# szlhl1040/Vehicles-Dispatch-Simulator

Measured on AMD Instinct MI355X. Metric: env-steps x replicas / sec (192-cluster, 10k vehicles), higher is better.
Workload: dtype int32

## Files before the change

### vehicles_dispatch_simulator_amd/csrc/vds_api.hip

```cpp
#include "../../include/vds.h"
#include "../../include/vds_debug.h"
#include "vds_device.h"
#include "vds_launch.h"

#include <algorithm>
#include <unordered_map>
#include <atomic>
#include <chrono>
#include <thread>
#include <cstdarg>
#include <cstdio>
#include <cstdlib>
#include <cstring>
#include <exception>
#include <map>
#include <mutex>
#include <new>
#include <numeric>
#include <string>
#include <vector>
#include <execinfo.h>
#include <signal.h>
#include <unistd.h>

// ... 1338 lines not shown
            for (int dd = 0; dd < n_days; ++dd) ok = ok && PD[dd].npull == ddesc[dd].Oq;
        if (!ok && S.dense_st) { S.dense = 0; S.dense_st = 0; }
        if (!ok) S.pull = 0;
        else {
            struct Sink2 { vds_handle *h; ~Sink2() { h->alloc_sink = nullptr; } } sink2{h};
            h->alloc_sink = &h->order_allocs;
            S.pull_W = W; S.pull_hmax = hmax;
            if ((rc = upload(h, &d, so_slot))) return rc; S.so_slot = d;
            int2 *d2; if ((rc = upload(h, &d2, d_rec))) return rc; S.d_rec = d2;
            if ((rc = upload(h, &d, d_first))) return rc; S.d_first = d;
            h->pull_desc = ddesc2;
            d_first_keep = d_first;
            h->pull_drec = std::move(d_rec);
            h->pull_slot_q.assign(h->pull_drec.size(), 0);
            for_each_day(n_days, [&](int dd) {
                const int qb = ddesc[dd].q_base;
                for (int q = qb; q < qb + ddesc[dd].Oq; ++q)
                    if (so_slot[q] >= 0) h->pull_slot_q[(size_t)ddesc2[dd].y + so_slot[q]] = q - qb;
            });
        }
    }
    h->pull_Od_max = Od_max;
    lt.lap("static arrival slots");
    S.tdesc = nullptr;
    if (S.dense && n_days == 1 && (int)h->corder_host.size() == C) {
        const DayDesc &de = ddesc[0];
        std::vector<int4> td((size_t)std::max(de.T, 1) * C * 2, make_int4(0, 0, 0, 0));
        std::vector<int4> cdd((size_t)C);
        HIPCHK(h, hipMemcpy(cdd.data(), S.cdesc_dense, (size_t)C * sizeof(int4), hipMemcpyDeviceToHost));
        for (int t = 0; t < de.T; ++t)
            for (int ci = 0; ci < C; ++ci) {
                const int c = h->corder_host[ci];
                const int q0 = bkt_off[de.bkt_base + (size_t)t * C + c], k = bkt_off[de.bkt_base + (size_t)t * C + c + 1] - q0;
                int clo = 0, n = 0;
                if (S.pull) {
                    clo = d_first_keep[(size_t)std::max(t - S.pull_W, 0) * C + c];
                    n = d_first_keep[(size_t)(t + 1) * C + c] - clo;
                }
                td[2 * ((size_t)t * C + ci)] = make_int4(q0, k, clo, n);
                td[2 * ((size_t)t * C + ci) + 1] = cdd[ci];
            }
        struct Sink3 { vds_handle *h; ~Sink3() { h->alloc_sink = nullptr; } } sink3{h};
        h->alloc_sink = &h->order_allocs;
        int4 *dtd; if ((rc = upload(h, &dtd, td))) return rc; S.tdesc = dtd;
    }
    h->alloc_sink = nullptr;
    lt.lap("bucket descriptors");
    if ((rc = apply_replica_map(h))) return rc;
    h->alloc_sink = nullptr;
    h->alloc_O = (int)std::min<long long>(Ototal / n_days, 0x7fffffff);
    if ((rc = alloc_state(h, h->alloc_O))) return rc;
    lt.lap("state tables");
    {
        const Static &Z = h->S;
        const int ids2 = std::max(Z.max_tick_orders, 4 * Z.C);
        const size_t lds2 = ((size_t)9 * Z.C + 1 + ids2 + ((size_t)Z.V + 2) / 2) * sizeof(int) + 2048;
        h->dfs2_ok = h->dfs_mode && Omax <= (1 << 20) && Z.max_nc <= 2047 && h->cost_min >= 0 && h->cost_max < (1 << 15) &&
                     Z.V <= 20480 && Z.N <= 65534 && Z.C <= 3072 && h->blk_ints < (1ll << 29) && Z.idle_cap <= 32767 && Z.max_tick_orders < 32768 &&
                     lds2 <= 64 * 1024;
        h->S.walk_pool = 0; h->S.walk_pool = dfs_walk_pool(h->S);
        h->hybrid_ok = h->dfs_mode && h->cfg.force_generic == 0 && Z.fast_ok && Z.max_nc * Z.max_nc <= h->lds_ints &&
                       Z.max_tick_orders < 65535 && Z.V < 65536 && Z.max_nc <= 2047 &&
                       Z.N <= 65534 && Z.C <= 65535 && Z.idle_cap <= 16384 && h->cost_max < (1 << 15) && h->max_seq <= 256 &&
                       dfs_walk_lds(Z) + 1024 <= 64 * 1024 && Z.so_vis != nullptr;
        if (Z.dense_st && !h->hybrid_ok)
            return fail(h, VDS_ECAPACITY, "vds_load_orders: neighbour search on the dense layout needs the walk's tables (idle_cap %d <= 16384, %zu bytes of LDS <= 64 KB); VDS_DENSE_DFS=0 keeps the wide layout",
                        Z.idle_cap, dfs_walk_lds(Z) + 1024);
// ... 1442 lines not shown
```

### vehicles_dispatch_simulator_amd/csrc/vds_device.h

```cpp
#pragma once
#include <hip/hip_runtime.h>
#include <stdint.h>

namespace vds {

enum {
    HDR_IDLE = 0,
    HDR_IDLE_PRE = 1,
    HDR_ORDERS = 2,
    HDR_FL = 3,
    HDR_INBOX0 = 4,
    HDR_INBOX1 = 5,
    HDR_RAW = 6,
    HDR_CNT32 = 8,
    HDR_WORDS = 16
};

enum {
    CNT_ORDERS = 0, CNT_REJECTS = 1, CNT_WAIT = 2, CNT_VALUE = 3,
    CNT_EVALS = 4, CNT_ARRIVALS = 5, CNT_DISPATCH = 6, CNT_DISPATCH_COST = 7, CNT_WORDS = 8
};

enum { ERR_IDLE_CAP = 1, ERR_FL_CAP = 2, ERR_INBOX_CAP = 4, ERR_DISPATCH = 8, ERR_RING_CAP = 16 };

// ... 67 lines not shown
    const unsigned char *so_lb;
    int seq_pad;
    const int *so_rank;
    int max_tick_orders;
    int r_lo;
    int dense;
    int dense_lpr;
    int dense_tab, dense_keys;
    int dense_force_slow;
    const Static *self_dev;
    const struct State *state_dev;
    int pull, pull_W, pull_hmax;
    int arr_slots;
    const int *so_slot;
    const int2 *d_rec;
    const int *d_first;
    const int4 *replica_desc2;
    int ring_min_on;
    const int *blk32s;
    const unsigned char *blk8s;
    const int4 *cdesc_dense;
    int dense_st;
    const int4 *tdesc;
};

struct Emit {
    hipStream_t st = nullptr;
    hipGraph_t graph = nullptr;
    const hipGraphNode_t *deps = nullptr;
    size_t ndeps = 0;
    hipGraphNode_t *node = nullptr;
    hipError_t *err = nullptr;
};
template <typename T> struct emit_arg { using type = T; };
template <typename... P>
static inline void emit_kernel(const Emit &e, void (*k)(P...), dim3 grid, dim3 block, size_t lds, typename emit_arg<P>::type... a) {
    if (!e.graph) { hipLaunchKernelGGL(k, grid, block, lds, e.st, a...); return; }
    void *args[] = {(void *)&a...};
    hipKernelNodeParams p{};
    p.func = reinterpret_cast<void *>(k); p.gridDim = grid; p.blockDim = block; p.sharedMemBytes = (unsigned)lds; p.kernelParams = args; p.extra = nullptr;
    *e.err = hipGraphAddKernelNode(e.node, e.graph, e.deps, e.ndeps, &p);
}

struct State {
    int *hdr;
    long long *cnt;
    uint2 *idle;
    int4 *ring;
    int *ring_cnt;
    int4 *fl;
    int4 *inbox;
    int4 *slog;
    int2 *out;
    int *err;
    int *work;
    unsigned *arr;
    unsigned short *stamp;
    int *slow_tick;
    int slow_T;
    int *dry;
    int *sup;
    int *sup_slot;
    int *ring_min;
};

#define DENSE_PULL_WMAX 3
#define VDS_SUP_PLANES 32
__host__ __device__ inline size_t sup_index(int C, int R, int slot, int c, int r) { return ((size_t)(slot & (VDS_SUP_PLANES - 1)) * C + c) * R + r; }
__host__ __device__ inline size_t arr_index(int R, int slot, int r) { return (size_t)slot * (size_t)R + (size_t)r; }
__host__ __device__ inline unsigned pull_entry(int veh, int arrival_slot) { return ((unsigned)veh << 8) | ((unsigned)arrival_slot & 0xFFu); }
__host__ __device__ inline unsigned pull_reject(int t) { return 0xFFFFFF00u | ((unsigned)(t + 128) & 0xFFu); }
__host__ __device__ inline bool pull_is_reject(unsigned e) { return (e >> 8) == 0xFFFFFFu; }
__host__ __device__ inline int pull_slots_ahead(unsigned e, int now_slot) { return (int)(signed char)((e & 0xFFu) - ((unsigned)now_slot & 0xFFu)); }
#define DENSE_DEAD_COST 0x00FFFFFF
#define DENSE_ID_BITS 25
__host__ __device__ inline unsigned dense_pack(unsigned veh, unsigned loc) { return (veh << 8) | (loc & 0xFFu); }
__host__ __device__ inline unsigned dense_key(int tick, int is_dispatch, int id) {
    return ((unsigned)(tick & 63) << 26) | ((unsigned)(is_dispatch & 1) << 25) | ((unsigned)id & ((1u << DENSE_ID_BITS) - 1));
}
__host__ __device__ inline unsigned dense_key_rel(unsigned key, int t) { return key - ((unsigned)((t - 32) & 63) << 26); }
__host__ __device__ inline int dense_key_is_dispatch(unsigned key) { return (int)((key >> 25) & 1u); }
__host__ __device__ inline int dense_key_id(unsigned key) { return (int)(key & ((1u << DENSE_ID_BITS) - 1)); }
__host__ __device__ inline int dense_key_tick(unsigned key, int t_now) { return t_now - (int)(((unsigned)t_now - (key >> 26)) & 63u); }

struct IdleRef {
    uint2 *p;
    unsigned *q;
    __device__ __forceinline__ uint2 get(int e) const {
        if (!q) return p[e];
// ... 29 lines not shown
```

### vehicles_dispatch_simulator_amd/csrc/vds_tick_dense.hip

```cpp
#include "vds_kernels_common.h"
#include "vds_launch.h"
#include <algorithm>

namespace vds {

VDS_PROF_ACCESSORS(dense)

#define SPAN_TICKS 256
#ifdef VDS_PROF
#define SPAN_WAYS 64
static __device__ unsigned long long g_span[2 * SPAN_TICKS * SPAN_WAYS * 2];
void read_span_dense(unsigned long long *out, int reset, hipStream_t st) {
    (void)hipStreamSynchronize(st);
    static unsigned long long host[2 * SPAN_TICKS * SPAN_WAYS * 2];
    if (out) {
        (void)hipMemcpyFromSymbol(host, HIP_SYMBOL(g_span), sizeof(host));
        for (int i = 0; i < 2 * SPAN_TICKS; ++i) {
            unsigned long long lo = ~0ull, hi = 0ull;
            for (int w = 0; w < SPAN_WAYS; ++w) { lo = std::min(lo, host[(i * SPAN_WAYS + w) * 2]); hi = std::max(hi, host[(i * SPAN_WAYS + w) * 2 + 1]); }
            out[2 * i] = lo; out[2 * i + 1] = hi;
        }
    }
    if (reset) {
        for (int i = 0; i < 2 * SPAN_TICKS * SPAN_WAYS; ++i) { host[2 * i] = ~0ull; host[2 * i + 1] = 0ull; }
// ... 2 lines not shown
}
#else
void read_span_dense(unsigned long long *, int, hipStream_t) { }
#endif

#define DN_ROWS 16
#define DN_TAB 128
#define DN_KEYS 64
#define DN_ORDERS 64
#ifndef DN_ROWS32
#define DN_ROWS32 1
#endif
#define DN_TPAD 4

struct DenseArgs {
    int *hdr; long long *cnt; unsigned *idle; uint2 *ring; int *ring_cnt; int4 *inbox; int2 *out; int *err;
    const int4 *cdesc_dense; const char *blk; const int4 *so_rec; const int *bkt_off; const int4 *replica_desc; const int *rperm;
    int R, C, H, idle_cap, ring_cap, in_cap, Oq, arr_slots;
    int tick_minutes, now0, tick_div_limit; unsigned tick_magic;
    int r_lo, r_hi, dense_tab, dense_keys, dense_force_slow;
    int *ring_min;
    unsigned *arr; const int *so_slot; const int2 *d_rec; const int *d_first; const int4 *replica_desc2; int pull_W;
    const int4 *tdesc;
    unsigned short *stamp; int *dry; int *slow_tick; const int *so_rank;
    int slow_T;
    const int2 *bmap;
    int *sup, *sup_slot;
    const Static *Sdev; const State *Ddev;
};
__device__ __forceinline__ uint2 *ring2(const DenseArgs &D) { return D.ring; }
__device__ __forceinline__ int ticks_until_fast(const DenseArgs &S, int rel) {
    const int n = rel + S.tick_minutes - 1;
    if (S.tick_div_limit > (1 << 26)) return (int)__umulhi((unsigned)n, S.tick_magic);
    return n / S.tick_minutes;
}

template <int LPR>
__device__ __forceinline__ int grp_min(int v) {
    v = min(v, dpp_mov<0xB1, 0xF>(v, v));
    v = min(v, dpp_mov<0x4E, 0xF>(v, v));
    if (LPR >= 8) v = min(v, dpp_mov<0x141, 0xF>(v, v));
    if (LPR >= 16) v = min(v, dpp_mov<0x140, 0xF>(v, v));
    return v;
}
template <int LPR>
__device__ __forceinline__ int grp_max(int v) {
// ... 482 lines not shown
            if (J >= 4) {
#pragma unroll
                for (int s = 0; s < J; s += 4) *reinterpret_cast<uint4 *>(tab + lbase + s) = make_uint4(e[s], e[s + 1], e[s + 2], e[s + 3]);
            } else {
                *reinterpret_cast<uint2 *>(tab + lbase) = make_uint2(e[0], e[1]);
            }
        }
        wave_order();
    }
#pragma unroll
    for (int a = 0; a < NAP; ++a)
        if (a * LPR + lg < A) tab[m + rank[a]] = ent[a];
    wave_order();
}
template <int LPR, int J>
__device__ __forceinline__ void pull_rank_place_any(const uint2 *ring, unsigned *tab, const int2 *drec, int lg, int m, int Ac, int A, int Amax, unsigned tbase, const unsigned *e,
                                                    bool cmp = false, unsigned am = 0u, int wp0 = 0) {
    if (Amax <= LPR) pull_rank_place<LPR, 1, J>(ring, tab, drec, lg, m, Ac, A, Amax, tbase, e, cmp, am, wp0);
    else if (Amax <= 2 * LPR) pull_rank_place<LPR, 2, J>(ring, tab, drec, lg, m, Ac, A, Amax, tbase, e, cmp, am, wp0);
    else if (Amax <= 4 * LPR || LPR == 16) pull_rank_place<LPR, 4, J>(ring, tab, drec, lg, m, Ac, A, Amax, tbase, e, cmp, am, wp0);
    else pull_rank_place<LPR, 8, J>(ring, tab, drec, lg, m, Ac, A, Amax, tbase, e, cmp, am, wp0);
}

template <int LPR>
__device__ __forceinline__ void store_counters(long long *cnt, int lg, long long cntv, int k, int rej, int wsum, int vsum, int evals, int A) {
#pragma unroll
    for (int w0 = 0; w0 < CNT_WORDS; w0 += LPR) {
        const int w = w0 + lg;
        long long d = 0;
        if (w == CNT_ORDERS) d = k;
        if (w == CNT_REJECTS) d = rej;
        if (w == CNT_WAIT) d = wsum;
        if (w == CNT_VALUE) d = vsum;
        if (w == CNT_EVALS) d = evals;
        if (w == CNT_ARRIVALS) d = A;
        if (LPR >= CNT_WORDS) { if (w < CNT_WORDS && d != 0) cnt[w] = cntv + d; }
        else if (d != 0) cnt[w] += d;
    }
}

template <bool RAW = false>
__device__ __forceinline__ void store_record(int *hdr, int lg, int2 hw, int idle, int pre, int orders, int rej, int wsum, int vsum, int evals, int A, int raw = 0) {
    if (lg == 0) hw = make_int2(idle, pre);
    if (lg == 1) hw.x = orders;
    if (RAW && lg == 3) hw.x = raw;
    if (lg == 4) { hw.x += orders; hw.y += rej; }
// ... 34 lines not shown
    for (int s = 0; s < J; ++s) e[s] = 0u;
    const bool dl = ST && m_raw != m;
    const bool anydl = ST && ballot(dl) != 0ull;
    if ((kmax > 0 || anydl) && lbase < (ST ? m_raw : m) && !(abl & 2048)) {
        if (J >= 4) {
#pragma unroll
            for (int s = 0; s < J; s += 4) {
                const uint4 v = *reinterpret_cast<const uint4 *>(idle + lbase + s);
                e[s] = v.x; e[s + 1] = v.y; e[s + 2] = v.z; e[s + 3] = v.w;
            }
        } else {
            const uint2 v = *reinterpret_cast<const uint2 *>(idle + lbase);
            e[0] = v.x; e[1] = v.y;
        }
    }
    PROF_STAMP(3);
    const int Amax = (abl & 2048) ? 0 : wave_max_of_groups<LPR>(PULL ? Aring : A);
    const int Ntot = PULL ? ((abl & 2048) ? 0 : wave_max_of_groups<LPR>(A)) : Amax;
#ifdef VDS_PROF
    if ((g_ablate & 2097152) && lane == 0) { atomicAdd(&D.err[12], 1); if (Ntot > 4 * LPR) atomicAdd(&D.err[13], 1); if (Ntot > 8 * LPR) atomicAdd(&D.err[14], 1); if (TS == 128) atomicAdd(&D.err[15], 1); }
#endif
    const unsigned tbase = (unsigned)((t - 32) & 63) << 26;
    const uint2 *ring = ring2(D) + si * S.ring_cap;
    unsigned am = 0u;
    if (ST) {
        const int nv = min(max(m_raw - lbase, 0), J);
        am = nv >= 32 ? 0xFFFFFFFFu : ((1u << nv) - 1u);
        if (dl && lbase < m_raw) {
            const unsigned *sp = reinterpret_cast<const unsigned *>(D.stamp + b * S.idle_cap + lbase);
            unsigned sw[(J + 1) / 2];
            if (J >= 8) {
#pragma unroll
                for (int s = 0; s < J / 2; s += 4) { const uint4 v = *reinterpret_cast<const uint4 *>(sp + s); sw[s] = v.x; sw[s + 1] = v.y; sw[s + 2] = v.z; sw[s + 3] = v.w; }
            } else if (J == 4) { const uint2 v = *reinterpret_cast<const uint2 *>(sp); sw[0] = v.x; sw[1] = v.y; }
            else sw[0] = sp[0];
            unsigned fm = 0u;
#pragma unroll
            for (int s = 0; s < J; ++s) fm |= (((sw[s >> 1] >> ((s & 1) << 4)) & 0xFFFFu) == 0xFFFFu ? 1u : 0u) << s;
            am &= fm;
        }
    }
    if (kmax == 0 && !anydl) {
        if (Ntot > 0) {
            if (PULL) pull_rank_place_any<LPR, 0>(ring, tab, lds_drec, lg, 0, A - Aring, A, Ntot, tbase, nullptr);
            else merge_arrivals_any<LPR, 0>(ring, tab, lg, 0, A, Amax, tbase, nullptr);
            if (rowvalid) {
                for (int idx = lg; idx < A; idx += LPR) { idle[m + idx] = tab[idx]; if (ST) D.stamp[b * S.idle_cap + m + idx] = (unsigned short)0xFFFFu; }
                if (lg == 0 && (PULL ? Aring : A) > 0) D.ring_cnt[si] = 0;
            }
        }
        if (rowvalid && lg == 2 && D.sup != nullptr) D.sup[(size_t)(t & (VDS_SUP_PLANES - 1)) * S.C * S.R + b] = 0;
        if (rowvalid) {
            if (REC && ST) store_record<true>(D.hdr + b * HDR_WORDS, lg, hw, mnew, mnew, 0, 0, 0, 0, 0, A, 0);
            else if (REC) store_record(D.hdr + b * HDR_WORDS, lg, hw, mnew, mnew, 0, 0, 0, 0, 0, A);
            else {
                if (lg < 3) D.hdr[b * HDR_WORDS + lg] = lg == HDR_ORDERS ? 0 : mnew;
                if (A > 0) store_counters<LPR>(D.cnt + b * CNT_WORDS, lg, cntv, 0, 0, 0, 0, 0, A);
            }
        }
        return;
    }
    int fdl = IMAX;
    if (ST && anydl) {
        const int na = __popc(am);
        const int wp0 = grp_incl_scan<LPR>(na, lg) - na;
        const int nv = min(max(m_raw - lbase, 0), J);
        const unsigned gone = ~am & (nv >= 32 ? 0xFFFFFFFFu : ((1u << nv) - 1u));
        fdl = grp_min<LPR>(gone ? lbase + __ffs((int)gone) - 1 : IMAX);
        if (Ntot > 0) pull_rank_place_any<LPR, J>(ring, tab, lds_drec, lg, m, A - Aring, A, Ntot, tbase, e, true, am, wp0);
        else {
            wave_order();
            int wp = wp0;
#pragma unroll
            for (int s = 0; s < J; ++s)
                if ((am >> s) & 1u) { tab[wp] = e[s]; ++wp; }
            wave_order();
        }
        if (rowvalid && lg == 0 && Aring > 0) D.ring_cnt[si] = 0;
        if (J >= 4) {
#pragma unroll
            for (int s = 0; s < J; s += 4) {
                const uint4 v = *reinterpret_cast<const uint4 *>(tab + lbase + s);
                e[s] = v.x; e[s + 1] = v.y; e[s + 2] = v.z; e[s + 3] = v.w;
            }
        } else {
            const uint2 v = *reinterpret_cast<const uint2 *>(tab + lbase);
            e[0] = v.x; e[1] = v.y;
        }
    } else
    if (Ntot > 0) {
        if (PULL) pull_rank_place_any<LPR, J>(ring, tab, lds_drec, lg, m, A - Aring, A, Ntot, tbase, e);
        else merge_arrivals_any<LPR, J>(ring, tab, lg, m, A, Amax, tbase, e);
        if (rowvalid && lg == 0 && (PULL ? Aring : A) > 0) D.ring_cnt[si] = 0;
        if (J >= 4) {
#pragma unroll
            for (int s = 0; s < J; s += 4) {
                const uint4 v = *reinterpret_cast<const uint4 *>(tab + lbase + s);
                e[s] = v.x; e[s + 1] = v.y; e[s + 2] = v.z; e[s + 3] = v.w;
            }
        } else {
            const uint2 v = *reinterpret_cast<const uint2 *>(tab + lbase);
            e[0] = v.x; e[1] = v.y;
        }
    }
    PROF_STAMP(4);
    const unsigned ncrep = (unsigned)nc * 0x01010101u;
    unsigned L[NL];
#pragma unroll
    for (int i = 0; i < NL; ++i) {
        unsigned v;
        if (J >= 4) v = loc_bytes4(e[4 * i], e[4 * i + 1], e[4 * i + 2], e[4 * i + 3]);
        else v = (e[0] & 0xFFu) | ((e[1] & 0xFFu) << 8) | (ncrep & 0xFFFF0000u);
        const int nv = min(max(mnew - lbase - 4 * i, 0), J >= 4 ? 4 : 2);
        const unsigned deadmask = (unsigned)(0xFFFFFFFFull << (8 * nv));
// ... 186 lines not shown
        if (REC && ST) store_record<true>(D.hdr + b * HDR_WORDS, lg, hw, mfin, mnew, k, rej, wsum, vsum, evals, A, mfin != mnew ? mnew + 1 : 0);
        else if (REC) store_record(D.hdr + b * HDR_WORDS, lg, hw, mfin, mnew, k, rej, wsum, vsum, evals, A);
        else {
            if (lg < 3) D.hdr[b * HDR_WORDS + lg] = lg == HDR_IDLE ? mfin : (lg == HDR_IDLE_PRE ? mnew : k);
            if (!(abl & 32768)) store_counters<LPR>(D.cnt + b * CNT_WORDS, lg, cntv, k, rej, wsum, vsum, evals, A);
        }
    }
    PROF_STAMP(8);
}

#ifndef DN_MIN_WAVES16
#define DN_MIN_WAVES16 8
#endif
#ifndef DN_MIN_WAVES8
#define DN_MIN_WAVES8 6
#endif
#ifndef DN_MIN_WAVES4
#define DN_MIN_WAVES4 4
#endif
#ifndef DN_MIN_WAVES256
#define DN_MIN_WAVES256 7
#endif

#define DN_CAND 128

template <bool U8, int DM, int LPR, bool PULL, int TABMAX, int ROWS, bool ST>
__device__ __forceinline__ void tick_dense_wg(const DenseArgs &P, int t, int ci, int row0, int tabl) {
    static_assert(TABMAX == 128 || (TABMAX == 256 && LPR == 16 && U8), "256-entry tables: 16 lanes per replica, byte costs");
    static_assert(!ST || (U8 && DM == 0 && PULL), "stamp form: byte costs, one shared day, static arrival slots");
    static_assert(ROWS == DN_ROWS || (ROWS == 32 && DM == 0 && LPR == 8) || ((ROWS == 8 || ROWS == 4) && DM == 1 && LPR == 16),
                  "32-row workgroups: one shared day, 8 lanes per replica; 8- / 4-row workgroups: one day per workgroup, 16 lanes per replica");
    const DenseArgs &S = P, &D = P;
#ifdef VDS_PROF
    const int span_i = (((P.r_lo != 0 ? 1 : 0) * SPAN_TICKS + (t & (SPAN_TICKS - 1))) * SPAN_WAYS + (int)(blockIdx.x & (SPAN_WAYS - 1))) * 2;
    if ((g_ablate & 1048576) && threadIdx.x == 0) atomicMin(&g_span[span_i], (unsigned long long)__builtin_amdgcn_s_memrealtime());
    struct SpanEnd { int i; __device__ ~SpanEnd() { if ((g_ablate & 1048576) && threadIdx.x == 0) atomicMax(&g_span[i + 1], (unsigned long long)__builtin_amdgcn_s_memrealtime()); } } span_end{span_i};
#endif
    if (DN_ABL & 512) return;
    if (blockIdx.x == 0 && threadIdx.x == 0 && P.sup_slot != nullptr) P.sup_slot[0] = (t + 1) & (VDS_SUP_PLANES - 1);
    typedef typename std::conditional<U8, unsigned char, int>::type CT;
    constexpr int RPW = WAVE / LPR;
    constexpr int NTHR = ROWS * LPR;
    extern __shared__ int lds_dyn[];
    int4 *lds_rec = reinterpret_cast<int4 *>(lds_dyn);
    int *lds_slot = reinterpret_cast<int *>(lds_rec + (DM == 2 ? DN_ROWS * DN_ORDERS * 2 / 16 : DN_ORDERS));
    int *lds_rank = lds_slot + (PULL ? DN_ORDERS : 0);
    int2 *lds_drec = reinterpret_cast<int2 *>(lds_rank + (ST ? DN_ORDERS : 0));
    unsigned *tab_all = reinterpret_cast<unsigned *>(lds_drec + (PULL ? DN_CAND : 0));
    CT *lds_blk = reinterpret_cast<CT *>(tab_all + ROWS * (TABMAX + DN_TPAD));
    int4 cd, td0 = make_int4(0, 0, 0, 0);
    if (DM == 0) {
        const int4 *tp = S.tdesc + 2 * ((size_t)t * S.C + ci);
        td0 = tp[0]; cd = tp[1];
    } else cd = S.cdesc_dense[ci];
    const int c = cd.z, nc = cd.x;
    const int wave = __builtin_amdgcn_readfirstlane((int)(threadIdx.x >> 6));
    const int lane = lane_id();
    const int g = lane / LPR, lg = lane & (LPR - 1);
    const int p = t & 1;
    const int rslot = row0 + wave * RPW + g;
    const int r = (DM == 1 && S.rperm != nullptr) ? S.rperm[rslot < S.r_hi ? rslot : S.r_lo] : rslot;
    bool rowvalid = rslot < S.r_hi && r >= 0 && r < S.R;
    unsigned short *pick = reinterpret_cast<unsigned short *>(lds_rec) + (wave * RPW + g) * DN_ORDERS;
#ifdef VDS_PROF
    const bool prof = (g_ablate & 128) != 0;
    unsigned long long tprev = prof ? __builtin_amdgcn_s_memtime() : 0ull;
#else
    const bool prof = false;
    unsigned long long tprev = 0ull;
#endif
    const int pwave = (int)((blockIdx.x * (NTHR / WAVE) + wave) & (PROF_WAVES - 1));
    int q0, k, now, qb = 0;
    int clo = 0, n = 0, qdb = 0;
    const int2 *drec_row = nullptr;
    if (DM == 2) {
        q0 = 0; k = 0; now = S.now0 + t * S.tick_minutes;
// ... 44 lines not shown
    const size_t b = (size_t)c * S.R + (rowvalid ? r : 0);
    const size_t si = (size_t)(t & (S.H - 1)) * S.C * S.R + b;
    const bool wg_ok = k <= DN_ORDERS && n <= DN_CAND;
    unsigned *tab = tab_all + (wave * RPW + g) * (TABMAX + DN_TPAD);
    int m = 0, far = 0, A = 0;
    long long cntv = 0;
    int4 h0 = make_int4(0, 0, 0, 0);
    int hin = 0, rcw = 0;
    int2 hw = make_int2(0, 0);
    if (rowvalid) {
        if (U8) { if (lg < 8) hw = *reinterpret_cast<const int2 *>(D.hdr + b * HDR_WORDS + 2 * lg); }
        else {
            h0 = *reinterpret_cast<const int4 *>(D.hdr + b * HDR_WORDS);
            hin = D.hdr[b * HDR_WORDS + HDR_INBOX0 + p];
            if (LPR >= CNT_WORDS && lg < CNT_WORDS && !(DN_ABL & 131072)) cntv = D.cnt[b * CNT_WORDS + lg];
        }
        rcw = D.ring_cnt[si];
    }
    const char *blk_g = S.blk + cd.y;
    const int4 *blk4 = reinterpret_cast<const int4 *>(blk_g);
    const int n4 = (nc * (nc + 1) * (int)sizeof(CT) + 15) >> 4;
    const bool stage = DM != 2 && k > 0;
    const bool mine = stage && (int)threadIdx.x < min(k, DN_ORDERS);
    const bool dmine = PULL && DM != 2 && wg_ok && (int)threadIdx.x < n;
    int4 sblk = make_int4(0, 0, 0, 0), srec = make_int4(0, 0, 0, 0);
    int sslot = -1, srank = 0;
    int2 sdrec = make_int2(0, 0);
    if (stage && (int)threadIdx.x < n4 && !(DN_ABL & 1024)) sblk = blk4[threadIdx.x];
    if (mine) { srec = S.so_rec[q0 + threadIdx.x]; if (PULL) sslot = S.so_slot[q0 + threadIdx.x]; if (ST) srank = S.so_rank[q0 + threadIdx.x]; }
    if (dmine) sdrec = S.d_rec[clo + threadIdx.x];
    int Ac = 0;
    if (PULL && wg_ok) {
        const unsigned *ar = D.arr + arr_index(S.R, clo - qdb, rowvalid ? r : 0);
        const unsigned never = pull_reject(t - 1);
        const int gsh = lane & ~(LPR - 1);
        constexpr int NIF = 4;
        for (int i0 = 0; i0 < n; i0 += NIF * LPR) {
            unsigned v[NIF];
#pragma unroll
            for (int u = 0; u < NIF; ++u) {
                const int idx = i0 + u * LPR + lg;
                v[u] = never;
                if (idx < n && rowvalid) v[u] = ar[(size_t)idx * S.R];
            }
#pragma unroll
            for (int u = 0; u < NIF; ++u) {
                const int idx = i0 + u * LPR + lg;
                const bool now_ = (v[u] & 0xFFu) == ((unsigned)t & 0xFFu);
                const unsigned gm = (unsigned)(ballot(now_) >> gsh) & ((1u << LPR) - 1u);
                const int pos = Ac + __popc(gm & ((1u << lg) - 1u));
                if (now_ && pos < DN_TH) { tab[pos] = v[u]; tab[DN_TH + pos] = (unsigned)idx; }
                Ac += __popc(gm);
            }
        }
    }
    asm volatile("" : "+v"(rcw));
    int Aring = rcw & 0xFFFF;
    A = Aring + Ac;
    int m_raw = 0;
    if (U8) {
        const int gb = (lane & ~(LPR - 1)) << 2;
        m = __builtin_amdgcn_ds_bpermute(gb, hw.x);
        far = __builtin_amdgcn_ds_bpermute(gb + 4, hw.y) | __builtin_amdgcn_ds_bpermute(gb + 8, p ? hw.y : hw.x);
        if (ST) { const int rw = __builtin_amdgcn_ds_bpermute(gb + 12, hw.x); m_raw = rw ? rw - 1 : m; }
    } else {
        m = h0.x;
        far = h0.w | hin;
    }
    if (DN_ABL & 256) { if (m + far + A + (int)cntv == 0x7FFFFFF1) D.err[1] = 1; return; }
    if (DM == 2) {
        int4 *lds4 = reinterpret_cast<int4 *>(lds_blk);
        for (int i = threadIdx.x; i < n4; i += NTHR) lds4[i] = blk4[i];
        if (wg_ok)
            for (int j = lg; j < k; j += LPR) pick[j] = (unsigned short)((S.so_rec[q0 + j].y & 0xFFFF) * (nc + 1));
    } else if (k > 0) {
        int4 *lds4 = reinterpret_cast<int4 *>(lds_blk);
        if (!(DN_ABL & 1024)) {
            if ((int)threadIdx.x < n4) lds4[threadIdx.x] = sblk;
            for (int i = threadIdx.x + NTHR; i < n4; i += NTHR) lds4[i] = blk4[i];
        }
        if (mine) { lds_rec[threadIdx.x] = srec; if (PULL) lds_slot[threadIdx.x] = sslot; if (ST) lds_rank[threadIdx.x] = srank; }
    }
    if (dmine) lds_drec[threadIdx.x] = sdrec;
    if (NTHR < DN_CAND && PULL && DM != 2 && wg_ok)
        for (int i = threadIdx.x + NTHR; i < n; i += NTHR) lds_drec[i] = S.d_rec[clo + i];
    PROF_STAMP(0);
    __syncthreads();
    PROF_STAMP_NW(1);
    const int mnew0 = ST ? max(m + A, m_raw) : m + A;
    const bool bad = rowvalid && (!wg_ok || far != 0 || Aring > S.dense_keys || Aring > S.ring_cap || A > DN_TAB || mnew0 > min(tabl, TABMAX) || mnew0 > S.idle_cap || S.dense_force_slow ||
                                  (PULL && (A - Aring > S.dense_keys * 2 || A > DN_TH)));
#ifdef VDS_PROF
    if (bad && lg == 0) {
        const int why = k > DN_ORDERS ? 4 : (n > DN_CAND ? 5 : (far != 0 ? 6 : ((Aring > S.dense_keys || Aring > S.ring_cap) ? 7 : (A > DN_TAB ? 8 : ((mnew0 > min(tabl, TABMAX) || mnew0 > S.idle_cap) ? 9 :
                        ((PULL && A - Aring > S.dense_keys * 2) ? 10 : 11))))));
        atomicAdd(&D.err[why], 1);
    }
#endif
    const unsigned long long badrows = ballot(bad && lg == 0);
    if (badrows != 0ull && lane == 0) {
        atomicAdd(&D.err[2], popc64(badrows));
        if (D.slow_tick != nullptr && t < D.slow_T) atomicAdd(&D.slow_tick[(size_t)t * S.C + c], popc64(badrows));
    }
    if (bad) { rowvalid = false; m = 0; A = 0; Aring = 0; }
    if (!rowvalid) m_raw = 0;
    const bool any = ballot(rowvalid) != 0;
    const int mmax = wave_max_of_groups<LPR>(ST ? max(m + A, m_raw) : m + A);
    PROF_STAMP_NW(2);
    if (any) {
        const int nn = (wg_ok && rowvalid) ? n : 0;
        const int kr = (DM == 2 && !rowvalid) ? 0 : k;
        const int kmax = DM == 2 ? wave_max_of_groups<LPR>(kr) : k;
        const int2 *drec = DM == 2 ? drec_row : lds_drec;
        const bool capable = ST && cd.w != 0;
        if (mmax <= 32) dense_body<LPR, 32, CT, DM, PULL, ST>(S, D, t, now, q0, kr, kmax, qb, lds_blk, nc, lds_rec, pick, tab, r, rowvalid, b, si, m, A, cntv, hw, nn, Aring, drec, lds_slot, prof, tprev, pwave, m_raw, capable, lds_rank);
        else if (mmax <= 64) dense_body<LPR, 64, CT, DM, PULL, ST>(S, D, t, now, q0, kr, kmax, qb, lds_blk, nc, lds_rec, pick, tab, r, rowvalid, b, si, m, A, cntv, hw, nn, Aring, drec, lds_slot, prof, tprev, pwave, m_raw, capable, lds_rank);
        else if (TABMAX <= 128 || mmax <= 128) dense_body<LPR, 128, CT, DM, PULL, ST>(S, D, t, now, q0, kr, kmax, qb, lds_blk, nc, lds_rec, pick, tab, r, rowvalid, b, si, m, A, cntv, hw, nn, Aring, drec, lds_slot, prof, tprev, pwave, m_raw, capable, lds_rank);
        else dense_body<LPR, (TABMAX > 128 ? 256 : 128), CT, DM, PULL, ST>(S, D, t, now, q0, kr, kmax, qb, lds_blk, nc, lds_rec, pick, tab, r, rowvalid, b, si, m, A, cntv, hw, nn, Aring, drec, lds_slot, prof, tprev, pwave, m_raw, capable, lds_rank);
    }
    for (unsigned long long rest = badrows; rest; rest &= rest - 1) {
        const int l0 = __ffsll((long long)rest) - 1;
        dense_bucket_slow<CT, ST>(*P.Sdev, *P.Ddev, c, rdlane(r, l0), t, reinterpret_cast<const CT *>(blk_g), nc, (DM == 2 || k > 0) ? lds_blk : (const CT *)nullptr);
    }
}

template <bool U8, int DM, int LPR, bool PULL, int TABMAX = DN_TAB, int ROWS = DN_ROWS, bool ST = false>
__global__ __launch_bounds__(ROWS * LPR, TABMAX > 128 ? DN_MIN_WAVES256 : (LPR == 16 ? DN_MIN_WAVES16 : (LPR == 8 ? DN_MIN_WAVES8 : DN_MIN_WAVES4))) void k_tick_dense(DenseArgs P, int t) {
    const int nchunks = gridDim.x / P.C;
    tick_dense_wg<U8, DM, LPR, PULL, TABMAX, ROWS, ST>(P, t, (int)(blockIdx.x / nchunks), P.r_lo + (int)(blockIdx.x % nchunks) * ROWS, P.dense_tab);
}

#ifndef DN_MIN_WAVES_MIX
#define DN_MIN_WAVES_MIX DN_MIN_WAVES8
#endif
template <bool ST>
__global__ __launch_bounds__(256, DN_MIN_WAVES_MIX) void k_tick_dense_mixed(DenseArgs P, int t) {
// ... 56 lines not shown
        if (S.blk8s) emit_kernel(e, k_tick_dense<true, 1, 16, PULL, DN_TAB, 8>, grid, dim3(8 * 16), lds, P, t);
        else emit_kernel(e, k_tick_dense<false, 1, 16, PULL, DN_TAB, 8>, grid, dim3(8 * 16), lds, P, t);
        return;
    }
    if (LPR == 16 && dm == 1 && S.row_gran == 4) {
        if (S.blk8s) emit_kernel(e, k_tick_dense<true, 1, 16, PULL, DN_TAB, 4>, grid, dim3(4 * 16), lds, P, t);
        else emit_kernel(e, k_tick_dense<false, 1, 16, PULL, DN_TAB, 4>, grid, dim3(4 * 16), lds, P, t);
        return;
    }
    if (S.blk8s) emit_kernel(e, dm == 2 ? k_tick_dense<true, 2, LPR, PULL> : (dm ? k_tick_dense<true, 1, LPR, PULL> : k_tick_dense<true, 0, LPR, PULL>), grid, block, lds, P, t);
    else emit_kernel(e, dm == 2 ? k_tick_dense<false, 2, LPR, PULL> : (dm ? k_tick_dense<false, 1, LPR, PULL> : k_tick_dense<false, 0, LPR, PULL>), grid, block, lds, P, t);
}

static DenseArgs dense_args(const Static &S, const State &D, int r_lo, int r_n) {
    DenseArgs P;
    P.hdr = D.hdr; P.cnt = D.cnt; P.idle = reinterpret_cast<unsigned *>(D.idle); P.ring = reinterpret_cast<uint2 *>(D.ring);
    P.ring_cnt = D.ring_cnt; P.inbox = D.inbox; P.out = D.out; P.err = D.err;
    P.cdesc_dense = S.cdesc_dense; P.blk = S.blk8s ? reinterpret_cast<const char *>(S.blk8s) : reinterpret_cast<const char *>(S.blk32s);
    P.so_rec = S.so_rec; P.bkt_off = S.bkt_off; P.replica_desc = S.replica_desc; P.rperm = S.rperm;
    P.arr_slots = S.arr_slots; P.R = S.R; P.C = S.C; P.H = S.H; P.idle_cap = S.idle_cap; P.ring_cap = S.ring_cap; P.in_cap = S.in_cap; P.Oq = S.Oq;
    P.tick_minutes = S.tick_minutes; P.now0 = S.now0; P.tick_div_limit = S.tick_div_limit; P.tick_magic = S.tick_magic;
    P.r_lo = r_lo; P.r_hi = r_lo + (r_n > 0 ? r_n : (S.rperm != nullptr ? S.rslots : S.R) - r_lo); P.dense_tab = S.dense_tab; P.dense_keys = S.dense_keys; P.dense_force_slow = S.dense_force_slow;
    P.Sdev = S.self_dev; P.Ddev = S.state_dev; P.ring_min = D.ring_min;
    P.tdesc = S.tdesc;
    P.stamp = D.stamp; P.dry = D.dry; P.slow_tick = D.slow_tick; P.so_rank = S.so_rank; P.sup = D.sup; P.sup_slot = D.sup_slot;
    P.arr = D.arr; P.so_slot = S.so_slot; P.d_rec = S.d_rec; P.d_first = S.d_first; P.replica_desc2 = S.replica_desc2; P.pull_W = S.pull_W;
    P.slow_T = D.slow_T; P.bmap = nullptr;
    return P;
}

static size_t dense_lds(const Static &S, int rows, int tab) {
    const int bb = (S.max_nc * (S.max_nc + 1) * (S.blk8s ? 1 : 4) + 15) / 16 * 16;
    return (S.n_days > 1 && !S.chunk_days ? DN_ROWS * DN_ORDERS * 2 : DN_ORDERS * 16) + (S.pull ? DN_ORDERS * 8 + DN_CAND * 8 : 0) + (S.dense_st ? DN_ORDERS * 4 : 0) +
           (size_t)rows * (tab + DN_TPAD) * 4 + bb;
}

bool dense_mixed_ok(const Static &S, int slots) {
    return S.dense && S.n_days <= 1 && S.blk8s != nullptr && S.pull && S.tdesc != nullptr && slots >= 64 && DN_ROWS32;
}

void emit_tick_dense_mixed(const Emit &e, const Static &S, const State &D, int t, const int2 *bmap, int nblk) {
    DenseArgs P = dense_args(S, D, 0, 0);
    P.bmap = bmap;
    const size_t lds = std::max(dense_lds(S, 32, DN_TAB), dense_lds(S, DN_ROWS, 256));
    if (S.dense_st) emit_kernel(e, k_tick_dense_mixed<true>, dim3(nblk), dim3(256), lds, P, t);
    else emit_kernel(e, k_tick_dense_mixed<false>, dim3(nblk), dim3(256), lds, P, t);
}

void emit_tick_dense(const Emit &e, const Static &S, const State &D, int t, int r_lo, int r_n) {
    const DenseArgs P = dense_args(S, D, r_lo, r_n);
    const int slots = r_n > 0 ? r_n : (S.rperm != nullptr ? S.rslots : S.R) - r_lo;
    const bool t256 = dense_tab256(S);
    const bool rows32 = S.n_days <= 1 && S.dense_lpr == 8 && !t256 && S.blk8s != nullptr && S.pull && slots >= 64 && DN_ROWS32;
    const bool rows8 = S.n_days > 1 && S.chunk_days && S.row_gran < 16 && S.dense_lpr == 16;
    const int rows = rows32 ? 32 : (rows8 ? S.row_gran : DN_ROWS);
    const int rchunks = (slots + rows - 1) / rows;
// ... 29 lines not shown
```

Baseline: 23.57 million.

## Precompute per-tick arrival order on host so dense pull kernel skips rank sort

Builds a host-side table that, for each tick and cluster, lists pull candidates already merged in arrival-key order. The single-day dense kernel reads candidates in that order, so arrivals land in the table sorted and the in-LDS rank/merge placement can be skipped when no ring entries exist. The per-workgroup staging of d_rec into LDS is also dropped for this mode, with reads going to global memory and the LDS budget shrinking. In exchange it adds host preprocessing at load time, an extra global table, and more gather-style reads from global memory.

```diff
diff --git a/profiles/r09_arrival_order/pmc_last_day.py b/profiles/r09_arrival_order/pmc_last_day.py
--- /dev/null
+++ b/profiles/r09_arrival_order/pmc_last_day.py
@@ -0,0 +1,15 @@
+import csv
+import glob
+import sys
+
+d, T = sys.argv[1], int(sys.argv[2])
+f = glob.glob(d + "/**/*counter_collection.csv", recursive=True)[0]
+per = {}
+for r in csv.DictReader(open(f)):
+    if "k_tick_dense" in r["Kernel_Name"]:
+        per.setdefault(int(r["Dispatch_Id"]), {})[r["Counter_Name"]] = float(r["Counter_Value"])
+last = [per[k] for k in sorted(per)[-T:]]
+tot = {c: sum(x.get(c, 0.0) for x in last) for c in ("SQ_INSTS_VALU", "SQ_INSTS_SALU", "SQ_INSTS_LDS", "SQ_WAVES")}
+w = tot["SQ_WAVES"]
+print("%d launches of the last day: %.0f wavefronts; per launch VALU %.2f M; per wavefront VALU %.1f SALU %.1f LDS %.1f"
+      % (len(last), w, tot["SQ_INSTS_VALU"] / len(last) / 1e6, tot["SQ_INSTS_VALU"] / w, tot["SQ_INSTS_SALU"] / w, tot["SQ_INSTS_LDS"] / w))
diff --git a/profiles/r09_arrival_order/reload_time.py b/profiles/r09_arrival_order/reload_time.py
--- /dev/null
+++ b/profiles/r09_arrival_order/reload_time.py
@@ -0,0 +1,14 @@
+import sys
+import time
+
+sys.path.insert(0, ".")
+from vehicles_dispatch_simulator_amd import workloads
+
+w = workloads.didi_day("cfg2")
+env = w.make_env(1024)
+env.reset(w.vehicle_nodes(1024))
+env.run(env.T); env.sync()
+ms = []
+for _ in range(6):
+    t0 = time.perf_counter(); env.load_orders(w.release_min, w.pickup, w.delivery); env.sync(); ms.append((time.perf_counter() - t0) * 1e3)
+print("load_orders on a loaded handle: first %.2f ms, then %s (mean %.2f ms)" % (ms[0], " ".join("%.2f" % m for m in ms[1:]), sum(ms[1:]) / 5))
diff --git a/vehicles_dispatch_simulator_amd/csrc/vds_api.hip b/vehicles_dispatch_simulator_amd/csrc/vds_api.hip
--- a/vehicles_dispatch_simulator_amd/csrc/vds_api.hip
+++ b/vehicles_dispatch_simulator_amd/csrc/vds_api.hip
@@ -1384,7 +1384,7 @@
     }
     h->pull_Od_max = Od_max;
     lt.lap("static arrival slots");
-    S.tdesc = nullptr;
+    S.tdesc = nullptr; S.d_ord = nullptr;
     if (S.dense && n_days == 1 && (int)h->corder_host.size() == C) {
         const DayDesc &de = ddesc[0];
         std::vector<int4> td((size_t)std::max(de.T, 1) * C * 2, make_int4(0, 0, 0, 0));
@@ -1405,6 +1405,37 @@
         struct Sink3 { vds_handle *h; ~Sink3() { h->alloc_sink = nullptr; } } sink3{h};
         h->alloc_sink = &h->order_allocs;
         int4 *dtd; if ((rc = upload(h, &dtd, td))) return rc; S.tdesc = dtd;
+        if (S.pull) {
+            pvec<unsigned short> ord((size_t)std::max(de.T, 1) * C * DENSE_CAND, (unsigned short)0);
+            const int2 *dr = h->pull_drec.data();
+            const int W = S.pull_W, nchunk = std::min(de.T, 16);
+            for_each_day(nchunk, [&](int ch) {
+                for (int t = (int)((long long)de.T * ch / nchunk); t < (int)((long long)de.T * (ch + 1) / nchunk); ++t)
+                    for (int ci = 0; ci < C; ++ci) {
+                        const int4 &b4 = td[2 * ((size_t)t * C + ci)];
+                        const int clo = b4.z, n = b4.w;
+                        if (n < 1 || n > DENSE_CAND) continue;
+                        const int c = h->corder_host[ci], alo = std::max(t - W, 0);
+                        int head[DENSE_PULL_WMAX + 2], end[DENSE_PULL_WMAX + 2];
+                        unsigned long long hk[DENSE_PULL_WMAX + 2];
+                        auto key_of = [&](int i) { const int2 r2 = dr[i]; return ((unsigned long long)(unsigned)((r2.y & 0xFFFF) - (int)((unsigned)r2.y >> 24)) << 32) | (unsigned)dense_key_id((unsigned)r2.x); };
+                        const int nr = t - alo + 1;
+                        for (int a = 0; a < nr; ++a) {
+                            head[a] = d_first_keep[(size_t)(alo + a) * C + c]; end[a] = d_first_keep[(size_t)(alo + a + 1) * C + c];
+                            hk[a] = head[a] < end[a] ? key_of(head[a]) : ~0ull;
+                        }
+                        unsigned short *o = ord.data() + ((size_t)t * C + ci) * DENSE_CAND;
+                        for (int i = 0; i < n; ++i) {
+                            int best = 0;
+                            for (int a = 1; a < nr; ++a) if (hk[a] < hk[best]) best = a;
+                            const int x = head[best]++;
+                            o[dense_ord_index(i)] = (unsigned short)((x - clo) | ((((unsigned)dr[x].y >> 16) & 0xFFu) << 8));
+                            hk[best] = head[best] < end[best] ? key_of(head[best]) : ~0ull;
+                        }
+                    }
+            });
+            unsigned short *dord; if ((rc = upload(h, &dord, ord))) return rc; S.d_ord = dord;
+        }
     }
     h->alloc_sink = nullptr;
     lt.lap("bucket descriptors");
diff --git a/vehicles_dispatch_simulator_amd/csrc/vds_device.h b/vehicles_dispatch_simulator_amd/csrc/vds_device.h
--- a/vehicles_dispatch_simulator_amd/csrc/vds_device.h
+++ b/vehicles_dispatch_simulator_amd/csrc/vds_device.h
@@ -113,6 +113,7 @@
     const int4 *cdesc_dense;
     int dense_st;
     const int4 *tdesc;
+    const unsigned short *d_ord;
 };
 
 struct Emit {
@@ -156,6 +157,8 @@
 };
 
 #define DENSE_PULL_WMAX 3
+#define DENSE_CAND 128
+__host__ __device__ inline int dense_ord_index(int i) { return (i & ~63) | ((i & 15) << 2) | ((i >> 4) & 3); }
 #define VDS_SUP_PLANES 32
 __host__ __device__ inline size_t sup_index(int C, int R, int slot, int c, int r) { return ((size_t)(slot & (VDS_SUP_PLANES - 1)) * C + c) * R + r; }
 __host__ __device__ inline size_t arr_index(int R, int slot, int r) { return (size_t)slot * (size_t)R + (size_t)r; }
diff --git a/vehicles_dispatch_simulator_amd/csrc/vds_tick_dense.hip b/vehicles_dispatch_simulator_amd/csrc/vds_tick_dense.hip
--- a/vehicles_dispatch_simulator_amd/csrc/vds_tick_dense.hip
+++ b/vehicles_dispatch_simulator_amd/csrc/vds_tick_dense.hip
@@ -48,6 +48,7 @@
     int *ring_min;
     unsigned *arr; const int *so_slot; const int2 *d_rec; const int *d_first; const int4 *replica_desc2; int pull_W;
     const int4 *tdesc;
+    const unsigned short *d_ord;
     unsigned short *stamp; int *dry; int *slow_tick; const int *so_rank;
     int slow_T;
     const int2 *bmap;
@@ -576,6 +577,108 @@
     else pull_rank_place<LPR, 8, J>(ring, tab, drec, lg, m, Ac, A, Amax, tbase, e, cmp, am, wp0);
 }
 
+template <int LPR, int NAP, int J>
+__device__ __forceinline__ void place_behind(unsigned *tab, int lg, int m, int A, const unsigned *e, bool cmp, unsigned am, int wp0, const unsigned *ent, const int *pos) {
+    if (J > 0) {
+        const int lbase = lg * J;
+        if (cmp) {
+            int wp = wp0;
+#pragma unroll
+            for (int s = 0; s < (J > 0 ? J : 1); ++s)
+                if ((am >> s) & 1u) { tab[wp] = e[s]; ++wp; }
+        } else if (lbase < m) {
+            if (J >= 4) {
+#pragma unroll
+                for (int s = 0; s < J; s += 4) *reinterpret_cast<uint4 *>(tab + lbase + s) = make_uint4(e[s], e[s + 1], e[s + 2], e[s + 3]);
+            } else {
+                *reinterpret_cast<uint2 *>(tab + lbase) = make_uint2(e[0], e[1]);
+            }
+        }
+        wave_order();
+    }
+#pragma unroll
+    for (int a = 0; a < NAP; ++a)
+        if (a * LPR + lg < A) tab[m + pos[a]] = ent[a];
+    wave_order();
+}
+template <int LPR, int NAP, int J>
+__device__ __forceinline__ void pull_place_sorted(unsigned *tab, int lg, int m, int A, const unsigned *e, bool cmp, unsigned am, int wp0) {
+    unsigned ent[NAP];
+    int pos[NAP];
+#pragma unroll
+    for (int a = 0; a < NAP; ++a) {
+        pos[a] = a * LPR + lg;
+        ent[a] = 0u;
+        if (pos[a] < A) ent[a] = tab[pos[a]];
+    }
+    wave_order();
+    place_behind<LPR, NAP, J>(tab, lg, m, A, e, cmp, am, wp0, ent, pos);
+}
+template <int LPR, int J>
+__device__ __forceinline__ void pull_place_sorted_any(unsigned *tab, int lg, int m, int A, int Amax, const unsigned *e, bool cmp = false, unsigned am = 0u, int wp0 = 0) {
+    if (Amax <= LPR) pull_place_sorted<LPR, 1, J>(tab, lg, m, A, e, cmp, am, wp0);
+    else if (Amax <= 2 * LPR) pull_place_sorted<LPR, 2, J>(tab, lg, m, A, e, cmp, am, wp0);
+    else if (Amax <= 4 * LPR || LPR == 16) pull_place_sorted<LPR, 4, J>(tab, lg, m, A, e, cmp, am, wp0);
+    else pull_place_sorted<LPR, 8, J>(tab, lg, m, A, e, cmp, am, wp0);
+}
+template <int LPR, int NAP, int J>
+__device__ __forceinline__ void pull_rank_place_hbm(const uint2 *ring, unsigned *tab, const int2 *drec, int lg, int m, int Ac, int A, int Amax, unsigned tbase, const unsigned *e,
+                                                    bool cmp, unsigned am, int wp0) {
+    unsigned key[NAP], ent[NAP];
+    int rank[NAP];
+#pragma unroll
+    for (int a = 0; a < NAP; ++a) {
+        const int idx = a * LPR + lg;
+        key[a] = 0xFFFFFFFFu; rank[a] = 0;
+        if (idx < Ac) key[a] = *reinterpret_cast<const unsigned *>(reinterpret_cast<const char *>(drec) + (tab[DN_TH + idx] << 3)) - tbase;
+        else if (idx < A) key[a] = ring[idx - Ac].y - tbase;
+    }
+    wave_order();
+#pragma unroll
+    for (int a = 0; a < NAP; ++a)
+        if (a * LPR + lg < Amax) tab[DN_TH + a * LPR + lg] = key[a];
+    wave_order();
+    for (int i = 0; i < Amax; ++i) {
+        const unsigned kk = tab[DN_TH + i];
+#pragma unroll
+        for (int a = 0; a < NAP; ++a) rank[a] += kk < key[a] ? 1 : 0;
+    }
+#pragma unroll
+    for (int a = 0; a < NAP; ++a) {
+        const int idx = a * LPR + lg;
+        ent[a] = 0u;
+        if (idx < Ac) ent[a] = tab[idx];
+        else if (idx < A) ent[a] = ring[idx - Ac].x;
+    }
+    wave_order();
+    place_behind<LPR, NAP, J>(tab, lg, m, A, e, cmp, am, wp0, ent, rank);
+}
+template <int LPR, int J>
+__device__ __forceinline__ void pull_rank_place_hbm_any(const uint2 *ring, unsigned *tab, const int2 *drec, int lg, int m, int Ac, int A, int Amax, unsigned tbase, const unsigned *e,
+                                                        bool cmp = false, unsigned am = 0u, int wp0 = 0) {
+    if (Amax <= LPR) pull_rank_place_hbm<LPR, 1, J>(ring, tab, drec, lg, m, Ac, A, Amax, tbase, e, cmp, am, wp0);
+    else if (Amax <= 2 * LPR) pull_rank_place_hbm<LPR, 2, J>(ring, tab, drec, lg, m, Ac, A, Amax, tbase, e, cmp, am, wp0);
+    else if (Amax <= 4 * LPR || LPR == 16) pull_rank_place_hbm<LPR, 4, J>(ring, tab, drec, lg, m, Ac, A, Amax, tbase, e, cmp, am, wp0);
+    else pull_rank_place_hbm<LPR, 8, J>(ring, tab, drec, lg, m, Ac, A, Amax, tbase, e, cmp, am, wp0);
+}
+
+template <int LPR>
+__device__ __forceinline__ void dord_load(const unsigned short *dord, int i0, int lg, unsigned (&w)[2]) {
+    static_assert(LPR == 16 || LPR == 8, "d_ord layout: 16 or 8 lanes per replica");
+    if (LPR == 16) {
+        const uint2 v = *reinterpret_cast<const uint2 *>(dord + i0 + lg * 4);
+        w[0] = v.x; w[1] = v.y;
+    } else {
+        const unsigned short *q = dord + (i0 & ~63) + ((i0 >> 5) & 1) * 2 + lg * 4;
+        w[0] = *reinterpret_cast<const unsigned *>(q);
+        w[1] = *reinterpret_cast<const unsigned *>(q + 32);
+    }
+}
+template <int LPR>
+__device__ __forceinline__ unsigned dord_entry(const unsigned (&w)[2], int u) {
+    return LPR == 16 ? (w[u >> 1] >> ((u & 1) << 4)) & 0xFFFFu : (w[u & 1] >> ((u >> 1) << 4)) & 0xFFFFu;
+}
+
 template <int LPR>
 __device__ __forceinline__ void store_counters(long long *cnt, int lg, long long cntv, int k, int rej, int wsum, int vsum, int evals, int A) {
 #pragma unroll
@@ -656,6 +759,7 @@
 #endif
     const unsigned tbase = (unsigned)((t - 32) & 63) << 26;
     const uint2 *ring = ring2(D) + si * S.ring_cap;
+    const bool sorted = PULL && DM == 0 && Amax == 0;
     unsigned am = 0u;
     if (ST) {
         const int nv = min(max(m_raw - lbase, 0), J);
@@ -676,7 +780,8 @@
     }
     if (kmax == 0 && !anydl) {
         if (Ntot > 0) {
-            if (PULL) pull_rank_place_any<LPR, 0>(ring, tab, lds_drec, lg, 0, A - Aring, A, Ntot, tbase, nullptr);
+            if (PULL && DM == 0) { if (!sorted) pull_rank_place_hbm_any<LPR, 0>(ring, tab, lds_drec, lg, 0, A - Aring, A, Ntot, tbase, nullptr); }
+            else if (PULL) pull_rank_place_any<LPR, 0>(ring, tab, lds_drec, lg, 0, A - Aring, A, Ntot, tbase, nullptr);
             else merge_arrivals_any<LPR, 0>(ring, tab, lg, 0, A, Amax, tbase, nullptr);
             if (rowvalid) {
                 for (int idx = lg; idx < A; idx += LPR) { idle[m + idx] = tab[idx]; if (ST) D.stamp[b * S.idle_cap + m + idx] = (unsigned short)0xFFFFu; }
@@ -701,7 +806,8 @@
         const int nv = min(max(m_raw - lbase, 0), J);
         const unsigned gone = ~am & (nv >= 32 ? 0xFFFFFFFFu : ((1u << nv) - 1u));
         fdl = grp_min<LPR>(gone ? lbase + __ffs((int)gone) - 1 : IMAX);
-        if (Ntot > 0) pull_rank_place_any<LPR, J>(ring, tab, lds_drec, lg, m, A - Aring, A, Ntot, tbase, e, true, am, wp0);
+        if (Ntot > 0 && sorted) pull_place_sorted_any<LPR, J>(tab, lg, m, A, Ntot, e, true, am, wp0);
+        else if (Ntot > 0) pull_rank_place_hbm_any<LPR, J>(ring, tab, lds_drec, lg, m, A - Aring, A, Ntot, tbase, e, true, am, wp0);
         else {
             wave_order();
             int wp = wp0;
@@ -723,7 +829,9 @@
         }
     } else
     if (Ntot > 0) {
-        if (PULL) pull_rank_place_any<LPR, J>(ring, tab, lds_drec, lg, m, A - Aring, A, Ntot, tbase, e);
+        if (PULL && sorted) pull_place_sorted_any<LPR, J>(tab, lg, m, A, Ntot, e);
+        else if (PULL && DM == 0) pull_rank_place_hbm_any<LPR, J>(ring, tab, lds_drec, lg, m, A - Aring, A, Ntot, tbase, e);
+        else if (PULL) pull_rank_place_any<LPR, J>(ring, tab, lds_drec, lg, m, A - Aring, A, Ntot, tbase, e);
         else merge_arrivals_any<LPR, J>(ring, tab, lg, m, A, Amax, tbase, e);
         if (rowvalid && lg == 0 && (PULL ? Aring : A) > 0) D.ring_cnt[si] = 0;
         if (J >= 4) {
@@ -956,7 +1064,7 @@
 #define DN_MIN_WAVES256 7
 #endif
 
-#define DN_CAND 128
+#define DN_CAND DENSE_CAND
 
 template <bool U8, int DM, int LPR, bool PULL, int TABMAX, int ROWS, bool ST>
 __device__ __forceinline__ void tick_dense_wg(const DenseArgs &P, int t, int ci, int row0, int tabl) {
@@ -980,12 +1088,19 @@
     int *lds_slot = reinterpret_cast<int *>(lds_rec + (DM == 2 ? DN_ROWS * DN_ORDERS * 2 / 16 : DN_ORDERS));
     int *lds_rank = lds_slot + (PULL ? DN_ORDERS : 0);
     int2 *lds_drec = reinterpret_cast<int2 *>(lds_rank + (ST ? DN_ORDERS : 0));
-    unsigned *tab_all = reinterpret_cast<unsigned *>(lds_drec + (PULL ? DN_CAND : 0));
+    unsigned *tab_all = reinterpret_cast<unsigned *>(lds_drec + ((PULL && DM != 0) ? DN_CAND : 0));
     CT *lds_blk = reinterpret_cast<CT *>(tab_all + ROWS * (TABMAX + DN_TPAD));
     int4 cd, td0 = make_int4(0, 0, 0, 0);
+    constexpr int NIF0 = 4;
+    unsigned ord0[2] = {0u, 0u};
+    const unsigned short *dord = nullptr;
     if (DM == 0) {
         const int4 *tp = S.tdesc + 2 * ((size_t)t * S.C + ci);
         td0 = tp[0]; cd = tp[1];
+        if (PULL) {
+            dord = S.d_ord + ((size_t)t * S.C + ci) * DN_CAND;
+            dord_load<LPR>(dord, 0, (int)(threadIdx.x & (LPR - 1)), ord0);
+        }
     } else cd = S.cdesc_dense[ci];
     const int c = cd.z, nc = cd.x;
     const int wave = __builtin_amdgcn_readfirstlane((int)(threadIdx.x >> 6));
@@ -1076,7 +1191,7 @@
     const int n4 = (nc * (nc + 1) * (int)sizeof(CT) + 15) >> 4;
     const bool stage = DM != 2 && k > 0;
     const bool mine = stage && (int)threadIdx.x < min(k, DN_ORDERS);
-    const bool dmine = PULL && DM != 2 && wg_ok && (int)threadIdx.x < n;
+    const bool dmine = PULL && DM == 1 && wg_ok && (int)threadIdx.x < n;
     int4 sblk = make_int4(0, 0, 0, 0), srec = make_int4(0, 0, 0, 0);
     int sslot = -1, srank = 0;
     int2 sdrec = make_int2(0, 0);
@@ -1088,22 +1203,32 @@
         const unsigned *ar = D.arr + arr_index(S.R, clo - qdb, rowvalid ? r : 0);
         const unsigned never = pull_reject(t - 1);
         const int gsh = lane & ~(LPR - 1);
-        constexpr int NIF = 4;
+        constexpr int NIF = NIF0;
         for (int i0 = 0; i0 < n; i0 += NIF * LPR) {
-            unsigned v[NIF];
+            unsigned v[NIF], o[NIF], ow[2];
+            if (DM == 0) {
+                ow[0] = ord0[0]; ow[1] = ord0[1];
+                if (i0 != 0) dord_load<LPR>(dord, i0, lg, ow);
+#pragma unroll
+                for (int u = 0; u < NIF; ++u) o[u] = dord_entry<LPR>(ow, u);
+            }
 #pragma unroll
             for (int u = 0; u < NIF; ++u) {
-                const int idx = i0 + u * LPR + lg;
+                const int sp = i0 + u * LPR + lg;
+                const int idx = DM == 0 ? (int)(o[u] & 0xFFu) : sp;
                 v[u] = never;
-                if (idx < n && rowvalid) v[u] = ar[(size_t)idx * S.R];
+                if (sp < n && rowvalid) v[u] = ar[(size_t)idx * S.R];
             }
 #pragma unroll
             for (int u = 0; u < NIF; ++u) {
-                const int idx = i0 + u * LPR + lg;
+                const int sp = i0 + u * LPR + lg;
                 const bool now_ = (v[u] & 0xFFu) == ((unsigned)t & 0xFFu);
                 const unsigned gm = (unsigned)(ballot(now_) >> gsh) & ((1u << LPR) - 1u);
                 const int pos = Ac + __popc(gm & ((1u << lg) - 1u));
-                if (now_ && pos < DN_TH) { tab[pos] = v[u]; tab[DN_TH + pos] = (unsigned)idx; }
+                if (now_ && pos < DN_TH) {
+                    tab[pos] = DM == 0 ? ((v[u] & 0xFFFFFF00u) | (o[u] >> 8)) : v[u];
+                    tab[DN_TH + pos] = DM == 0 ? (o[u] & 0xFFu) : (unsigned)sp;
+                }
                 Ac += __popc(gm);
             }
         }
@@ -1136,7 +1261,7 @@
         if (mine) { lds_rec[threadIdx.x] = srec; if (PULL) lds_slot[threadIdx.x] = sslot; if (ST) lds_rank[threadIdx.x] = srank; }
     }
     if (dmine) lds_drec[threadIdx.x] = sdrec;
-    if (NTHR < DN_CAND && PULL && DM != 2 && wg_ok)
+    if (NTHR < DN_CAND && PULL && DM == 1 && wg_ok)
         for (int i = threadIdx.x + NTHR; i < n; i += NTHR) lds_drec[i] = S.d_rec[clo + i];
     PROF_STAMP(0);
     __syncthreads();
@@ -1165,7 +1290,7 @@
         const int nn = (wg_ok && rowvalid) ? n : 0;
         const int kr = (DM == 2 && !rowvalid) ? 0 : k;
         const int kmax = DM == 2 ? wave_max_of_groups<LPR>(kr) : k;
-        const int2 *drec = DM == 2 ? drec_row : lds_drec;
+        const int2 *drec = DM == 2 ? drec_row : (DM == 0 ? S.d_rec + clo : lds_drec);
         const bool capable = ST && cd.w != 0;
         if (mmax <= 32) dense_body<LPR, 32, CT, DM, PULL, ST>(S, D, t, now, q0, kr, kmax, qb, lds_blk, nc, lds_rec, pick, tab, r, rowvalid, b, si, m, A, cntv, hw, nn, Aring, drec, lds_slot, prof, tprev, pwave, m_raw, capable, lds_rank);
         else if (mmax <= 64) dense_body<LPR, 64, CT, DM, PULL, ST>(S, D, t, now, q0, kr, kmax, qb, lds_blk, nc, lds_rec, pick, tab, r, rowvalid, b, si, m, A, cntv, hw, nn, Aring, drec, lds_slot, prof, tprev, pwave, m_raw, capable, lds_rank);
@@ -1268,7 +1393,7 @@
     P.tick_minutes = S.tick_minutes; P.now0 = S.now0; P.tick_div_limit = S.tick_div_limit; P.tick_magic = S.tick_magic;
     P.r_lo = r_lo; P.r_hi = r_lo + (r_n > 0 ? r_n : (S.rperm != nullptr ? S.rslots : S.R) - r_lo); P.dense_tab = S.dense_tab; P.dense_keys = S.dense_keys; P.dense_force_slow = S.dense_force_slow;
     P.Sdev = S.self_dev; P.Ddev = S.state_dev; P.ring_min = D.ring_min;
-    P.tdesc = S.tdesc;
+    P.tdesc = S.tdesc; P.d_ord = S.d_ord;
     P.stamp = D.stamp; P.dry = D.dry; P.slow_tick = D.slow_tick; P.so_rank = S.so_rank; P.sup = D.sup; P.sup_slot = D.sup_slot;
     P.arr = D.arr; P.so_slot = S.so_slot; P.d_rec = S.d_rec; P.d_first = S.d_first; P.replica_desc2 = S.replica_desc2; P.pull_W = S.pull_W;
     P.slow_T = D.slow_T; P.bmap = nullptr;
@@ -1277,7 +1402,7 @@
 
 static size_t dense_lds(const Static &S, int rows, int tab) {
     const int bb = (S.max_nc * (S.max_nc + 1) * (S.blk8s ? 1 : 4) + 15) / 16 * 16;
-    return (S.n_days > 1 && !S.chunk_days ? DN_ROWS * DN_ORDERS * 2 : DN_ORDERS * 16) + (S.pull ? DN_ORDERS * 8 + DN_CAND * 8 : 0) + (S.dense_st ? DN_ORDERS * 4 : 0) +
+    return (S.n_days > 1 && !S.chunk_days ? DN_ROWS * DN_ORDERS * 2 : DN_ORDERS * 16) + (S.pull ? DN_ORDERS * 8 + (S.n_days > 1 ? DN_CAND * 8 : 0) : 0) + (S.dense_st ? DN_ORDERS * 4 : 0) +
            (size_t)rows * (tab + DN_TPAD) * 4 + bb;
 }
 
```

New measurement: 23.58 million, median of 4. Within noise of the previous version (+0.1%).
